# zjkang/Relation-DETR

Hardware: AMD Instinct MI355X
Metric: images/sec @ 800×1333, 300 queries, R50 4-level; achieved HBM GB/s (higher is better)
Workload: dtype bf16; 1 GPU; relation_detr_resnet50_800_1333 transformer stack from feature pyramids: 6 encoder layers (MSDA self-attn, S=22323, 4 levels) + two-stage top-k + 6 decoder layers (relation-biased self-attn + MSDA cross-attn + box refinement) + top-300 detections; backbone/neck excluded; batch_per_gpu=4, global_batch=4, queries=900, levels=4, launch=hipGraph replay, streams=2, gemm_tuning=False, parallelism=image-parallel x1

## Files before the change

include/relation_detr_amd.h:

```cpp
#ifndef RELATION_DETR_AMD_H
#define RELATION_DETR_AMD_H

#include <stdint.h>

#ifdef __cplusplus
extern "C" {
#endif

#define RDETR_ABI_VERSION 3

typedef enum rdetr_status {
    RDETR_OK = 0,
    RDETR_ERR_INVALID_ARG = -1,
    RDETR_ERR_UNSUPPORTED = -2,
    RDETR_ERR_LAUNCH = -3
} rdetr_status;

int rdetr_abi_version(void);
const char *rdetr_status_string(int status);

int rdetr_msda_forward_f32(const float *value, const int64_t *spatial_shapes, const int64_t *level_start_index,
                           const float *sampling_loc, const float *attn_weight, int B, int S, int H, int D,
                           int L, int Nq, int P, float *out, void *stream);

// ... 219 lines not shown
int rdetr_query_pos_inproj_k256_bf16(const uint16_t *emb, long long lde, const uint16_t *query, long long ldq, const uint16_t *pw1a,
                                     const uint16_t *pw1b, const uint16_t *b1, const uint16_t *pw2, const uint16_t *b2, const uint16_t *pv1,
                                     const uint16_t *c1, const uint16_t *pv2, const uint16_t *c2, const uint16_t *pwq, const uint16_t *pwk,
                                     const uint16_t *pwv, const uint16_t *bias, long long M, uint16_t *out_pos, uint16_t *out_qpp,
                                     uint16_t *out_qk, long long ldqk, uint16_t *out_v, long long ldv, void *stream);

int rdetr_encoder_proj_k256_bf16(const uint16_t *x, long long ldx, const uint16_t *xq, long long ldq, const uint16_t *pwv,
                                 const uint16_t *bv, const uint16_t *pwq, const uint16_t *bq, const uint8_t *row_mask, int B, int S,
                                 int q_cols, uint16_t *out_hm, uint16_t *out_q, void *stream);

int rdetr_detections_from_topk(const float *score, const long long *index, const float *boxes, const long long *image_sizes, int B,
                               int N, int C, int K, float *out, void *stream);

int rdetr_scaled_pos(const void *a, const void *scale, const void *query, long long n, int is_bf16, void *pos, void *qp, void *stream);

int rdetr_decoder_reference(const float *reference, const float *valid_ratios, int B, int N, int L, int F, float temperature,
                            float scale, float *ref_in, void *emb, int emb_is_bf16, void *stream);

int rdetr_pyramid_points(const unsigned char *const *level_masks, const int *level_hw, int L, int B, const unsigned char *pad_mask,
                         int keep_is_bf16, float *valid_ratios, float *reference, float *logit, void *keep, void *stream);
int rdetr_nchw_to_tokens(const void *src, const void *add_vec, int is_bf16, int B, int C, int P,
                         long long out_image_stride, long long ld_out, void *out, void *stream);
int rdetr_nchw_levels_to_tokens(const void *const *level_src, const void *const *level_vec, const int *level_pixels, int L,
                                int is_bf16, int B, int C, long long out_image_stride, long long ld_out, void *out, void *stream);

int rdetr_linear_k256_bf16(const uint16_t *x, long long ldx, const uint16_t *w, const uint16_t *bias, long long M, int N,
                           int relu, uint16_t *out, long long ldo, void *stream);

int rdetr_linear_pack_k256_bf16(const uint16_t *w, uint16_t *packed, void *stream);
int rdetr_linear_ln_k256_bf16(const uint16_t *x, long long ldx, const uint16_t *packed, const uint16_t *bias,
                              const uint16_t *residual, long long ldr, const uint16_t *gamma, const uint16_t *beta, float eps,
                              long long M, uint16_t *out, long long ldo, void *stream);

int rdetr_ffn_k256_pack_bf16(const uint16_t *w1, const uint16_t *w2, int F, uint16_t *packed, void *stream);
int rdetr_ffn_k256_bf16(const uint16_t *x, long long ldx, const uint16_t *packed, const uint16_t *b1, const uint16_t *b2,
                        long long M, int F, uint16_t *out, long long ldo, void *stream);
int rdetr_ffn_ln_k256_bf16(const uint16_t *x, long long ldx, const uint16_t *packed, const uint16_t *b1, const uint16_t *b2,
                           const uint16_t *gamma, const uint16_t *beta, float eps, const uint16_t *pos, long long ldp,
                           long long M, int F, uint16_t *out, long long ldo, uint16_t *out2, long long ldo2, void *stream);
int rdetr_ffn_k256_train_bf16(const uint16_t *x, long long ldx, const uint16_t *packed, const uint16_t *b1, const uint16_t *b2,
                              long long M, int F, uint16_t *out, long long ldo, uint16_t *hid, long long ldh, void *stream);
int rdetr_ffn_k256_backward_bf16(const uint16_t *dy, long long lddy, const uint16_t *packed_t, const uint16_t *hid, long long ldh,
                                 long long M, int F, uint16_t *dh, long long ldd, uint16_t *dx, long long lddx, void *stream);
int rdetr_ffn_k256_pack_f32(const float *w1, long long w1_row_stride, long long w1_col_stride, const float *w2,
                            long long w2_row_stride, long long w2_col_stride, const float *b1, const float *b2, int F,
                            uint16_t *packed, uint16_t *biases_bf16, void *stream);
int rdetr_ffn_k256_train_xf32_bf16(const float *x, long long ldx, const uint16_t *packed, const uint16_t *b1, const uint16_t *b2,
                                   long long M, int F, uint16_t *out, long long ldo, uint16_t *hid, long long ldh, uint16_t *xlp,
                                   long long ldxl, void *stream);
int rdetr_ffn_k256_backward_dxf32_bf16(const uint16_t *dy, long long lddy, const uint16_t *packed_t, const uint16_t *hid,
                                       long long ldh, long long M, int F, uint16_t *dh, long long ldd, float *dx, long long lddx,
                                       void *stream);

int rdetr_match_cost_f32(const float *logits, long long ld_logits, const float *boxes, long long ld_boxes, const float *gt_boxes,
                         const int *gt_labels, const int *gt_count, int R, int B, int N, int C, int Gmax, float alpha, float gamma,
                         float w_class, float w_bbox, float w_giou, float *cost, void *stream);
int rdetr_match_cost_bf16(const uint16_t *logits, long long ld_logits, const float *boxes, long long ld_boxes, const float *gt_boxes,
                          const int *gt_labels, const int *gt_count, int R, int B, int N, int C, int Gmax, float alpha, float gamma,
                          float w_class, float w_bbox, float w_giou, float *cost, void *stream);
long long rdetr_set_loss_workspace_bytes(int R, int N);
int rdetr_set_loss_f32(const float *logits, long long ld_logits, const float *boxes, long long ld_boxes, const int *match,
                       const float *gt_boxes, const int *gt_labels, int R, int B, int N, int C, int Gmax, int n_split, float inv_norm_a,
                       float inv_norm_b, float alpha, float gamma, void *ws, long long ws_bytes, float *sums, float *dlogits,
                       float *dbox_l1, float *dbox_giou, void *stream);
int rdetr_set_loss_bf16(const uint16_t *logits, long long ld_logits, const float *boxes, long long ld_boxes, const int *match,
                        const float *gt_boxes, const int *gt_labels, int R, int B, int N, int C, int Gmax, int n_split, float inv_norm_a,
// ... 43 lines not shown
```

relation_detr_amd/_lib.py:

```python
from __future__ import annotations

import ctypes
import os

_HERE = os.path.dirname(os.path.abspath(__file__))
LIB_PATH = os.environ.get("RDETR_LIB_PATH") or os.path.join(_HERE, "librelation_detr_amd.so")

_c_int, _c_float, _vp, _c_ll = ctypes.c_int, ctypes.c_float, ctypes.c_void_p, ctypes.c_longlong
_c_ull = ctypes.c_ulonglong

SIGNATURES = {
    "rdetr_abi_version": [],
    "rdetr_status_string": [_c_int],
    "rdetr_msda_fast_path": [_c_int] * 4,
    "rdetr_msda_levels_window_ok": [_vp, _vp, _c_int, _c_ll],
    "rdetr_msda_forward_f32": [_vp] * 5 + [_c_int] * 7 + [_vp, _vp],
    "rdetr_msda_forward_bf16": [_vp] * 5 + [_c_int] * 7 + [_vp, _vp],
    "rdetr_msda_forward_fused_f32": [_vp] * 6 + [_c_int] * 8 + [_vp, _vp],
    "rdetr_msda_forward_fused_bf16": [_vp] * 6 + [_c_int] * 8 + [_vp, _vp],
    "rdetr_msda_forward_fused_ex_f32": [_vp] * 4 + [_c_int, _vp, _c_int, _vp, _c_int, _vp] + [_c_int] * 7 + [_vp, _vp],
    "rdetr_msda_forward_fused_ex_bf16": [_vp] * 4 + [_c_int, _vp, _c_int, _vp, _c_int, _vp] + [_c_int] * 7 + [_vp, _vp],
    "rdetr_msda_forward_opt_bf16": [_vp, _c_int] + [_vp] * 4 + [_c_int] * 8 + [_vp, _vp],
    "rdetr_msda_forward_sweep_bf16": [_vp, _c_int] + [_vp] * 4 + [_c_int] * 7 + [_vp, _vp],
    "rdetr_msda_forward_resident_bf16": [_vp] * 5 + [_c_int] * 7 + [_vp, _vp],
# ... 15 lines not shown
    "rdetr_relation_bias_backward_f32": [_vp] * 4 + [_c_int] * 5 + [_c_float] * 3 + [_vp] * 4,
    "rdetr_bias_softmax_f32": [_vp] * 3 + [_c_int] * 3 + [_vp],
    "rdetr_relation_attention_bf16": [_vp] * 3 + [_c_int] * 3 + [_vp, _vp] + [_c_int] * 5 + [_c_float, _vp, _c_int, _vp],
    "rdetr_relation_attention_train_bf16": [_vp] * 3 + [_c_int] * 3 + [_vp, _vp] + [_c_int] * 5 + [_c_float, _vp, _c_int, _vp, _vp],
    "rdetr_relation_attention_backward_workspace_bytes": [_c_int] * 3,
    "rdetr_relation_attention_backward_bf16": [_vp] * 3 + [_c_int] * 3 + [_vp, _c_int, _vp, _vp, _c_int, _vp, _vp] + [_c_int] * 5
                                              + [_c_float, _vp, _c_ll] + [_vp, _c_int] * 3 + [_vp, _vp],
    "rdetr_relation_attention_boxes_bf16": [_vp] * 3 + [_c_int] * 3 + [_vp] * 5 + [_c_int] * 6 + [_c_float] * 4 + [_vp, _c_int, _vp],
    "rdetr_relation_attention_boxes_train_bf16": [_vp] * 3 + [_c_int] * 3 + [_vp] * 5 + [_c_int] * 6 + [_c_float] * 4
                                                 + [_vp, _c_int, _vp, _vp],
    "rdetr_relation_attention_boxes_backward_workspace_bytes": [_c_int] * 4,
    "rdetr_relation_attention_boxes_backward_bf16": [_vp] * 3 + [_c_int] * 3 + [_vp, _c_int, _vp, _vp, _c_int] + [_vp] * 5 + [_c_int] * 6
                                                    + [_c_float] * 4 + [_vp, _c_ll] + [_vp, _c_int] * 3 + [_vp, _vp, _vp],
    "rdetr_box_refine_f32": [_vp, _c_int, _vp, _c_ll, _c_float, _vp, _vp],
    "rdetr_sine_pos_embed": [_vp, _c_ll, _c_int, _c_int, _c_float, _c_float, _vp, _c_int, _vp],
    "rdetr_zero_masked_rows": [_vp, _vp, _c_ll, _c_int, _c_ll, _vp],
    "rdetr_row_max": [_vp, _c_int, _c_ll, _c_int, _c_ll, _vp, _vp],
    "rdetr_topk_workspace_bytes": [_c_int, _c_int, _c_int],
    "rdetr_topk": [_vp, _c_int, _c_int, _c_int, _c_int, _vp, _vp, _vp, _vp],
    "rdetr_box_head_k256_bf16": [_vp, _c_ll, _vp, _c_ll, _vp, _vp, _vp, _vp, _vp, _vp, _vp, _c_int, _c_float, _c_ll, _vp, _vp, _vp],
    "rdetr_box_head_cls_k256_bf16": [_vp, _c_ll, _vp, _c_ll, _vp, _vp, _vp, _vp, _vp, _vp, _vp, _c_int, _c_float, _vp, _vp, _c_int, _c_ll,
                                     _vp, _vp, _vp, _c_ll, _vp],
    "rdetr_query_pos_k256_bf16": [_vp, _c_ll, _vp, _c_ll] + [_vp] * 9 + [_c_ll, _vp, _vp, _vp],
    "rdetr_query_pos_inproj_k256_bf16": [_vp, _c_ll, _vp, _c_ll] + [_vp] * 13 + [_c_ll, _vp, _vp, _vp, _c_ll, _vp, _c_ll, _vp],
    "rdetr_encoder_proj_k256_bf16": [_vp, _c_ll, _vp, _c_ll] + [_vp] * 5 + [_c_int, _c_int, _c_int, _vp, _vp, _vp],
    "rdetr_detections_from_topk": [_vp, _vp, _vp, _vp, _c_int, _c_int, _c_int, _c_int, _vp, _vp],
    "rdetr_scaled_pos": [_vp, _vp, _vp, _c_ll, _c_int, _vp, _vp, _vp],
    "rdetr_decoder_reference": [_vp, _vp, _c_int, _c_int, _c_int, _c_int, _c_float, _c_float, _vp, _vp, _c_int, _vp],
    "rdetr_pyramid_points": [_vp, _vp, _c_int, _c_int, _vp, _c_int, _vp, _vp, _vp, _vp, _vp],
    "rdetr_linear_k256_bf16": [_vp, _c_ll, _vp, _vp, _c_ll, _c_int, _c_int, _vp, _c_ll, _vp],
    "rdetr_linear_k256_hm_bf16": [_vp, _c_ll, _vp, _vp, _vp, _c_int, _c_int, _vp, _vp],
    "rdetr_linear_pack_k256_bf16": [_vp, _vp, _vp],
    "rdetr_linear_ln_k256_bf16": [_vp, _c_ll, _vp, _vp, _vp, _c_ll, _vp, _vp, _c_float, _c_ll, _vp, _c_ll, _vp],
    "rdetr_ffn_k256_pack_bf16": [_vp, _vp, _c_int, _vp, _vp],
    "rdetr_ffn_k256_bf16": [_vp, _c_ll, _vp, _vp, _vp, _c_ll, _c_int, _vp, _c_ll, _vp],
    "rdetr_ffn_ln_k256_bf16": [_vp, _c_ll, _vp, _vp, _vp, _vp, _vp, _c_float, _vp, _c_ll, _c_ll, _c_int, _vp, _c_ll, _vp, _c_ll, _vp],
    "rdetr_ffn_k256_train_bf16": [_vp, _c_ll, _vp, _vp, _vp, _c_ll, _c_int, _vp, _c_ll, _vp, _c_ll, _vp],
    "rdetr_ffn_k256_backward_bf16": [_vp, _c_ll, _vp, _vp, _c_ll, _c_ll, _c_int, _vp, _c_ll, _vp, _c_ll, _vp],
    "rdetr_ffn_k256_pack_f32": [_vp, _c_ll, _c_ll, _vp, _c_ll, _c_ll, _vp, _vp, _c_int, _vp, _vp, _vp],
    "rdetr_ffn_k256_train_xf32_bf16": [_vp, _c_ll, _vp, _vp, _vp, _c_ll, _c_int, _vp, _c_ll, _vp, _c_ll, _vp, _c_ll, _vp],
    "rdetr_ffn_k256_backward_dxf32_bf16": [_vp, _c_ll, _vp, _vp, _c_ll, _c_ll, _c_int, _vp, _c_ll, _vp, _c_ll, _vp],
    "rdetr_nchw_to_tokens": [_vp, _vp, _c_int, _c_int, _c_int, _c_int, _c_ll, _c_ll, _vp, _vp],
    "rdetr_nchw_levels_to_tokens": [_vp, _vp, _vp, _c_int, _c_int, _c_int, _c_int, _c_ll, _c_ll, _vp, _vp],
    "rdetr_add_layernorm_f32": [_vp] * 4 + [_c_ll, _c_int, _c_float, _vp, _vp],
    "rdetr_add_layernorm_bf16": [_vp] * 4 + [_c_ll, _c_int, _c_float, _vp, _vp],
    "rdetr_add_layernorm_strided_f32": [_vp] * 4 + [_c_ll, _c_int, _c_ll, _c_ll, _c_ll, _c_float, _vp, _vp],
    "rdetr_add_layernorm_strided_bf16": [_vp] * 4 + [_c_ll, _c_int, _c_ll, _c_ll, _c_ll, _c_float, _vp, _vp],
    "rdetr_add_layernorm_pos_f32": [_vp] * 5 + [_c_ll, _c_int] + [_c_ll] * 5 + [_c_float, _vp, _vp, _vp],
    "rdetr_add_layernorm_pos_bf16": [_vp] * 5 + [_c_ll, _c_int] + [_c_ll] * 5 + [_c_float, _vp, _vp, _vp],
    "rdetr_add_layernorm_train_f32": [_vp] * 4 + [_c_ll, _c_int, _c_ll, _c_ll, _c_ll, _c_float, _vp, _vp, _vp],
    "rdetr_add_layernorm_train_bf16": [_vp] * 4 + [_c_ll, _c_int, _c_ll, _c_ll, _c_ll, _c_float, _vp, _vp, _vp],
    "rdetr_add_layernorm_backward_workspace_bytes": [_c_ll],
    "rdetr_add_layernorm_backward_f32": [_vp, _c_ll] * 3 + [_vp, _vp, _c_ll, _c_int, _vp, _c_ll] + [_vp] * 4,
    "rdetr_add_layernorm_backward_bf16": [_vp, _c_ll] * 3 + [_vp, _vp, _c_ll, _c_int, _vp, _c_ll] + [_vp] * 4,
    "rdetr_add_layernorm_train_mixed": [_vp, _c_int, _c_ll, _vp, _c_int, _c_ll, _vp, _vp, _c_ll, _c_int, _c_float, _vp, _c_ll, _vp, _vp],
    "rdetr_add_layernorm_backward_mixed": [_vp, _c_ll, _vp, _c_int, _c_ll, _vp, _c_int, _c_ll, _vp, _vp, _c_ll, _c_int, _vp, _c_ll]
                                          + [_vp] * 5,
    "rdetr_match_cost_f32": [_vp, _c_ll, _vp, _c_ll, _vp, _vp, _vp] + [_c_int] * 5 + [_c_float] * 5 + [_vp, _vp],
    "rdetr_match_cost_bf16": [_vp, _c_ll, _vp, _c_ll, _vp, _vp, _vp] + [_c_int] * 5 + [_c_float] * 5 + [_vp, _vp],
    "rdetr_set_loss_workspace_bytes": [_c_int, _c_int],
    "rdetr_set_loss_f32": [_vp, _c_ll, _vp, _c_ll, _vp, _vp, _vp] + [_c_int] * 6 + [_c_float] * 4 + [_vp, _c_ll] + [_vp] * 5,
    "rdetr_set_loss_bf16": [_vp, _c_ll, _vp, _c_ll, _vp, _vp, _vp] + [_c_int] * 6 + [_c_float] * 4 + [_vp, _c_ll] + [_vp] * 5,
    "rdetr_cdn_queries_f32": [_vp] * 3 + [_c_int] * 6 + [_c_float] * 2 + [_vp] * 5 + [_c_int, _c_ull] + [_vp] * 4,
    "rdetr_cdn_queries_bf16": [_vp] * 3 + [_c_int] * 6 + [_c_float] * 2 + [_vp] * 5 + [_c_int, _c_ull] + [_vp] * 4,
    "rdetr_cdn_mask": [_c_int] * 3 + [_vp, _vp],
    "rdetr_cdn_embed_backward_f32": [_vp, _vp] + [_c_int] * 3 + [_vp, _vp],
# ... 41 lines not shown
```

relation_detr_amd/ms_deform_attn.py:

```python
from __future__ import annotations

import math
import warnings

import torch
from torch import Tensor, nn

from . import amp_train, ln_train, msda_train_hm, ops
from . import options as _options


def sampling_locations(reference_points: Tensor, offsets: Tensor, spatial_shapes: Tensor, num_points: int) -> Tensor:
    last = reference_points.shape[-1]
    if last == 2:
        wh = spatial_shapes.flip(-1).to(offsets.dtype)
        return reference_points[:, :, None, :, None, :] + offsets / wh[None, None, None, :, None, :]
    if last == 4:
        centre = reference_points[:, :, None, :, None, :2]
        size = reference_points[:, :, None, :, None, 2:]
        return centre + offsets / num_points * size * 0.5
    raise ValueError("Last dim of reference_points must be 2 or 4, but get {} instead.".format(last))


class MultiScaleDeformableAttention(nn.Module):
    def __init__(self, embed_dim: int = 256, num_levels: int = 4, num_heads: int = 8, num_points: int = 4,
                 img2col_step: int = 64):
        super().__init__()
        if embed_dim % num_heads != 0:
            raise ValueError(
                "embed_dim must be divisible by num_heads, but got {} and {}".format(embed_dim, num_heads))
        head_dim = embed_dim // num_heads
        if head_dim & (head_dim - 1):
            warnings.warn("head_dim is not a power of two; the wave-per-query HIP kernel needs head_dim == 32, "
                          "other sizes run the generic kernel")
        self.im2col_step = img2col_step
        self.embed_dim = embed_dim
        self.num_heads = num_heads
        self.num_levels = num_levels
        self.num_points = num_points
        self.options = _options.get()
        self.sampling_offsets = nn.Linear(embed_dim, num_heads * num_levels * num_points * 2)
# ... 138 lines not shown
                and ops.msda_fast_path(self.num_heads, self.embed_dim // self.num_heads, self.num_levels, self.num_points)):
            core = ops.ms_deform_attn_forward_fused(
                v.to(core_dtype).contiguous(), spatial_shapes, level_start_index, offsets.to(core_dtype).contiguous(),
                logits.to(core_dtype).contiguous(), reference_points.float().contiguous())
        elif (needs_grad and self.options.msda_train_fused and v.is_cuda and core_dtype in (torch.float32, torch.bfloat16)
                and ops.msda_fast_path(self.num_heads, self.embed_dim // self.num_heads, self.num_levels, self.num_points)):
            core = ops.MultiScaleDeformableAttnFusedFunction.apply(
                v.to(core_dtype).contiguous(), spatial_shapes, level_start_index, offsets.to(core_dtype).contiguous(),
                logits.to(core_dtype).contiguous(), reference_points.float().contiguous())
        else:
            weights = logits.softmax(-1).view(*offsets.shape[:5])
            loc = sampling_locations(reference_points, offsets, spatial_shapes, self.num_points)
            core = ops.MultiScaleDeformableAttnFunction.apply(
                v.to(core_dtype).contiguous(), spatial_shapes, level_start_index, loc.float().contiguous(),
                weights.float().contiguous(), self.im2col_step)
        return self._output(core, vdt, post_norm)

    def _trains_head_major(self, query: Tensor, reference_points: Tensor, value: Tensor) -> bool:
        if not (self.options.msda_train_head_major and self.options.value_head_major and torch.is_grad_enabled() and value.is_cuda):
            return False
        so, aw, vp = self.sampling_offsets, self.attention_weights, self.value_proj
        if not (value.dtype == torch.bfloat16 and query.dtype == torch.bfloat16 and reference_points.shape[-1] == 2
                and query.shape[1] == value.shape[1] and value.shape[1] >= 4096 and value.dim() == 3 and query.shape[0] == value.shape[0]
                and all(m.weight.dtype == torch.bfloat16 for m in (so, aw, vp)) and so.bias is not None and aw.bias is not None
                and ops.msda_fast_path(self.num_heads, self.embed_dim // self.num_heads, self.num_levels, self.num_points)):
            return False
        return any(t.requires_grad for t in (query, value, reference_points, *so.parameters(), *aw.parameters(), *vp.parameters()))

    def _output(self, core: Tensor, vdt, post_norm) -> Tensor:
        if core.dtype != vdt:
            core = core.to(vdt)
        if post_norm is None:
            return self.output_proj(core)
        residual, norm = post_norm
        if (core.is_cuda and not torch.is_grad_enabled() and core.numel() // core.shape[-1] >= 16384
                and self.options.proj_ln and norm.weight is not None and norm.bias is not None
                and ops.linear_ln_k256_supported(core, self.output_proj.weight, residual)):
            return ops.linear_ln_k256(core, self.output_proj.weight, self.output_proj.bias, residual, norm.weight, norm.bias, norm.eps)
        out = self.output_proj(core)
        if out.is_cuda and not torch.is_grad_enabled() and out.dtype in (torch.float32, torch.bfloat16):
            return ops.add_layer_norm(out, residual, norm.weight, norm.bias, norm.eps)
        if (self.options.ln_train_fused and torch.is_grad_enabled()
                and (out.requires_grad or residual.requires_grad or (norm.weight is not None and norm.weight.requires_grad))):
            if ln_train.add_layer_norm_train_supported(out, residual, norm.weight, norm.bias):
                return ln_train.AddLayerNormFunction.apply(out, residual, norm.weight, norm.bias, norm.eps)
            if amp_train.autocast_bf16_active() and amp_train.add_layer_norm_mixed_supported(out, residual, norm.weight, norm.bias):
                return amp_train.AddLayerNormMixedFunction.apply(out, residual, norm.weight, norm.bias, norm.eps)
        return norm(residual + out)
```

relation_detr_amd/ops.py:

```python
from __future__ import annotations

import collections
import weakref
from typing import Optional, Tuple

import torch

from . import _lib


_KEEP: "collections.deque" = collections.deque(maxlen=64)


def _cptr(t: torch.Tensor) -> int:
    if t.is_contiguous():
        return t.data_ptr()
    c = t.contiguous()
    _KEEP.append(c)
    return c.data_ptr()


def _stream_ptr(t: torch.Tensor) -> int:
    return torch.cuda.current_stream(t.device).cuda_stream


def _require_device(*tensors: torch.Tensor) -> None:
    for t in tensors:
        if t is not None and not t.is_cuda:
            raise _lib.RdetrError(
                "relation_detr_amd operators need tensors on a ROCm device (got a CPU tensor); "
                "there is no CPU fallback on the product path")


def _require_contiguous(**named: torch.Tensor) -> None:
    for name, t in named.items():
        if t is not None and not t.is_contiguous():
            raise _lib.RdetrError(f"{name} tensor has to be contiguous")


_shape_cache: dict = {}

# ... 1303 lines not shown
    out2, ldp = None, 0
    if pos is not None:
        if tuple(pos.shape) != tuple(x.shape) or pos.dtype != x.dtype:
            raise _lib.RdetrError("ffn_ln_k256: pos must have x's shape and dtype")
        prows, _, ldp = _rows_view(pos, "ffn_ln_k256")
        if ldp % 8 or pos.data_ptr() % 16:
            raise _lib.RdetrError("ffn_ln_k256: pos rows must be 16-byte aligned")
        out2 = torch.empty(*x.shape[:-1], 256, dtype=x.dtype, device=x.device)
    packed = ffn_k256_packed_weights(w1, w2)
    st = _lib.load().rdetr_ffn_ln_k256_bf16(x.data_ptr(), ldx, packed.data_ptr(), _cptr(b1), _cptr(b2),
                                            _cptr(gamma), _cptr(beta), float(eps),
                                            None if pos is None else pos.data_ptr(), ldp, rows, F, out.data_ptr(), ldo,
                                            None if out2 is None else out2.data_ptr(), 256, _stream_ptr(x))
    _lib.check(st, "rdetr_ffn_ln_k256_bf16")
    return out if pos is None else (out, out2)


_LINEAR_PACKED = _PackedWeightCache()
_REL_PROJ_F32 = _PackedWeightCache()


def linear_ln_k256_supported(x: torch.Tensor, weight: torch.Tensor, residual: torch.Tensor) -> bool:
    if not (linear_k256_supported(x, weight) and tuple(weight.shape) == (256, 256) and residual.dtype == torch.bfloat16
            and residual.is_cuda and tuple(residual.shape) == tuple(x.shape)):
        return False
    try:
        _, _, ldr = _rows_view(residual, "linear_ln_k256")
    except _lib.RdetrError:
        return False
    return ldr % 8 == 0 and residual.data_ptr() % 16 == 0


def linear_ln_k256(x: torch.Tensor, weight: torch.Tensor, bias: Optional[torch.Tensor], residual: torch.Tensor,
                   gamma: torch.Tensor, beta: torch.Tensor, eps: float = 1e-5, out: Optional[torch.Tensor] = None) -> torch.Tensor:
    _require_device(x, weight, bias, residual, gamma, beta, out)
    if not linear_ln_k256_supported(x, weight, residual):
        raise _lib.RdetrError("linear_ln_k256: needs bf16 [..., 256] inputs with evenly strided 16-byte aligned rows and a [256, 256] weight")
    for t in (bias, gamma, beta):
        if t is not None and (t.dtype != torch.bfloat16 or t.numel() != 256):
            raise _lib.RdetrError("linear_ln_k256: bias / gamma / beta must be bf16 [256]")
    rows, _, ldx = _rows_view(x, "linear_ln_k256")
    _, _, ldr = _rows_view(residual, "linear_ln_k256")
    if out is None:
        out = torch.empty(x.shape, dtype=x.dtype, device=x.device)
    elif tuple(out.shape) != tuple(x.shape) or out.dtype != x.dtype:
        raise _lib.RdetrError("linear_ln_k256: out must have x's shape and dtype")
    orows, _, ldo = _rows_view(out, "linear_ln_k256")
    if orows != rows or ldo % 8 or out.data_ptr() % 16:
        raise _lib.RdetrError("linear_ln_k256: out rows must be 16-byte aligned")
    lib = _lib.load()
    def build():
        packed = torch.empty(256 * 256, dtype=torch.bfloat16, device=weight.device)
        _lib.check(lib.rdetr_linear_pack_k256_bf16(weight.data_ptr(), packed.data_ptr(), _stream_ptr(weight)), "rdetr_linear_pack_k256_bf16")
        if not torch.cuda.is_current_stream_capturing():
            torch.cuda.current_stream(weight.device).synchronize()
        return packed
    packed_w = _LINEAR_PACKED.get((weight,), build)
    st = lib.rdetr_linear_ln_k256_bf16(x.data_ptr(), ldx, packed_w.data_ptr(), None if bias is None else _cptr(bias),
                                       residual.data_ptr(), ldr, _cptr(gamma), _cptr(beta),
                                       float(eps), rows, out.data_ptr(), ldo, _stream_ptr(x))
    _lib.check(st, "rdetr_linear_ln_k256_bf16")
    return out
```

relation_detr_amd/self_attn.py:

```python
from __future__ import annotations

import math
from typing import Optional

import torch
from torch import Tensor, nn
from torch.nn import functional as F

from . import ops, options
from .attn_rel_train import RelationAttentionBoxesFunction
from .relation import DeferredRelationBias


class _BiasSoftmaxFunction(torch.autograd.Function):
    @staticmethod
    def forward(ctx, scores, bias, mask):
        probs = ops.bias_softmax_(scores, bias, mask)
        ctx.save_for_backward(probs)
        ctx.has_bias = bias is not None
        ctx.mark_dirty(scores)
        return probs

    @staticmethod
    @torch.autograd.function.once_differentiable
    def backward(ctx, grad):
        (p,) = ctx.saved_tensors
        gs = p * (grad - (grad * p).sum(-1, keepdim=True))
        return gs, (gs if ctx.has_bias else None), None


class RelationSelfAttention(nn.Module):

    def __init__(self, embed_dim: int, num_heads: int, dropout: float = 0.0, batch_first: bool = True):
        super().__init__()
        if not batch_first:
            raise NotImplementedError("the reference only uses batch_first=True (relation_transformer.py:406-408)")
        if embed_dim % num_heads:
            raise ValueError("embed_dim must be divisible by num_heads")
        self.embed_dim, self.num_heads, self.head_dim = embed_dim, num_heads, embed_dim // num_heads
        self.dropout = dropout
        self.batch_first = True
        self.in_proj_weight = nn.Parameter(torch.empty(3 * embed_dim, embed_dim))
        self.in_proj_bias = nn.Parameter(torch.zeros(3 * embed_dim))
        self.out_proj = nn.Linear(embed_dim, embed_dim)
        nn.init.xavier_uniform_(self.in_proj_weight)
        nn.init.zeros_(self.out_proj.bias)
        self.options = options.get()

    def forward(self, query: Tensor, key: Tensor, value: Tensor, attn_mask: Optional[Tensor] = None,
                need_weights: bool = False, key_padding_mask: Optional[Tensor] = None, projected=None):
        if need_weights or key_padding_mask is not None:
            raise NotImplementedError("need_weights / key_padding_mask are not used on this path")
        B, N, C = query.shape
        M = key.shape[1]
        H, d = self.num_heads, self.head_dim
        v = None
        if (projected is not None and key is query and not torch.is_grad_enabled() and query.dtype == torch.bfloat16
                and all(torch.is_tensor(t) and t.dtype == torch.bfloat16 and t.device == query.device for t in projected)
                and tuple(projected[0].shape) == (B, N, 2 * C) and tuple(projected[1].shape) == (B, M, C)):
            qk, v = projected
            q, k = qk[..., :C], qk[..., C:]
        elif key is query:
            qk = F.linear(query, self.in_proj_weight[:2 * C], self.in_proj_bias[:2 * C])
            q, k = qk[..., :C], qk[..., C:]
        else:
            q = F.linear(query, self.in_proj_weight[:C], self.in_proj_bias[:C])
            k = F.linear(key, self.in_proj_weight[C:2 * C], self.in_proj_bias[C:2 * C])
        if v is None:
            v = F.linear(value, self.in_proj_weight[2 * C:], self.in_proj_bias[2 * C:])
        needs_grad = torch.is_grad_enabled() and (q.requires_grad or k.requires_grad or v.requires_grad)
        if isinstance(attn_mask, DeferredRelationBias):
            rel = attn_mask
            conv = rel.module.pos_proj[0]
            if (q.is_cuda and q.dtype == torch.bfloat16 and d == 32 and H == 8 and rel.module.num_pos_feats == 16 and not needs_grad
                    and not (torch.is_grad_enabled() and conv.weight.requires_grad)
                    and tuple(rel.src_boxes.shape) == (B, N, 4) and tuple(rel.tgt_boxes.shape) == (B, M, 4)
                    and (rel.attn_mask is None or rel.attn_mask.dtype == torch.bool and tuple(rel.attn_mask.shape) == (N, M))):
                ctx = ops.relation_attention_boxes(q, k, v, H, rel.src_boxes, rel.tgt_boxes, conv.weight, conv.bias, rel.attn_mask,
                                                   1.0 / math.sqrt(d), rel.module.num_pos_feats, rel.module.temperature,
                                                   rel.module.scale)
                return self.out_proj(ctx), None
            if (self.options.rel_train_fused and torch.is_grad_enabled() and (needs_grad or conv.weight.requires_grad)
                    and q.is_cuda and q.dtype == torch.bfloat16 and k.dtype == torch.bfloat16 and v.dtype == torch.bfloat16
                    and d == 32 and H == 8 and rel.module.num_pos_feats == 16 and (self.dropout == 0.0 or not self.training)
                    and tuple(rel.src_boxes.shape) == (B, N, 4) and tuple(rel.tgt_boxes.shape) == (B, M, 4)
                    and (rel.attn_mask is None or rel.attn_mask.dtype == torch.bool and tuple(rel.attn_mask.shape) == (N, M))):
                packed = key is query
                ctx = RelationAttentionBoxesFunction.apply(
                    qk if packed else q, None if packed else k, v, rel.src_boxes, rel.tgt_boxes, conv.weight, conv.bias, rel.attn_mask,
                    H, 1.0 / math.sqrt(d), rel.module.num_pos_feats, rel.module.temperature, rel.module.scale)
                return self.out_proj(ctx), None
            attn_mask = rel.materialize()
        if (needs_grad and self.options.attn_train_fused and q.is_cuda and q.dtype == torch.bfloat16 and k.dtype == torch.bfloat16
                and v.dtype == torch.bfloat16 and d == 32 and (self.dropout == 0.0 or not self.training)
                and (attn_mask is None or attn_mask.dtype == torch.bool and tuple(attn_mask.shape) == (N, M)
                     or attn_mask.dtype != torch.bool and attn_mask.numel() == B * H * N * M)):
            is_bool = attn_mask is not None and attn_mask.dtype == torch.bool
            bias = None if attn_mask is None or is_bool else attn_mask.float().reshape(B * H, N, M)
            mask = attn_mask if is_bool else None
            if key is query:
                ctx = ops.RelationAttentionFunction.apply(qk, None, v, bias, mask, H, 1.0 / math.sqrt(d))
            else:
                ctx = ops.RelationAttentionFunction.apply(q, k, v, bias, mask, H, 1.0 / math.sqrt(d))
            return self.out_proj(ctx), None
        if (q.is_cuda and q.dtype == torch.bfloat16 and d == 32 and not needs_grad
                and (attn_mask is None or attn_mask.dtype == torch.bool and attn_mask.dim() == 2
                     or attn_mask.dtype != torch.bool and attn_mask.numel() == B * H * N * M)):
            is_bool = attn_mask is not None and attn_mask.dtype == torch.bool
            ctx = ops.relation_attention(q, k, v, H, None if attn_mask is None or is_bool else attn_mask.float(),
                                         attn_mask if is_bool else None, 1.0 / math.sqrt(d))
            return self.out_proj(ctx), None
        q = (q * (1.0 / math.sqrt(d))).view(B, N, H, d).transpose(1, 2).contiguous()
        k = k.view(B, M, H, d).transpose(1, 2).contiguous()
        v = v.view(B, M, H, d).transpose(1, 2).contiguous()
        scores = torch.matmul(q, k.transpose(-1, -2)).float().reshape(B * H, N, M).contiguous()
        bias = mask = None
        if attn_mask is not None:
            if attn_mask.dtype == torch.bool:
                if attn_mask.dim() != 2:
                    raise NotImplementedError("boolean attn_mask must be [N, N]")
                mask = attn_mask
            else:
                bias = attn_mask.float().reshape(B * H, N, M)
        probs = _BiasSoftmaxFunction.apply(scores, bias, mask)
        if self.dropout > 0.0 and self.training:
            probs = F.dropout(probs, self.dropout)
        ctx = torch.matmul(probs.view(B, H, N, M).to(v.dtype), v).transpose(1, 2).reshape(B, N, C)
        return self.out_proj(ctx), None
```

relation_detr_amd/transformer.py:

```python
from __future__ import annotations

import math
from typing import List, Sequence

import torch
from torch import Tensor, nn
from torch.nn import functional as F

from . import amp_train, ffn_train, ln_train, ops
from . import options as _options
from .ms_deform_attn import MultiScaleDeformableAttention
from .relation import PositionRelationEmbedding
from .self_attn import RelationSelfAttention


def inverse_sigmoid(x: Tensor, eps: float = 1e-3) -> Tensor:
    x = x.clamp(min=0, max=1)
    return torch.log(x.clamp(min=eps) / (1 - x).clamp(min=eps))


def refine_boxes(delta: Tensor, reference: Tensor) -> Tensor:
    if delta.is_cuda and reference.dtype == torch.float32 and not (torch.is_grad_enabled() and delta.requires_grad):
        from . import ops
        return ops.box_refine(delta, reference)
    return (delta.float() + inverse_sigmoid(reference)).sigmoid()


def sine_pos_embed(pos: Tensor, num_pos_feats: int = 128, temperature: float = 10000.0,
                   scale: float = 2 * math.pi) -> Tensor:
    k = torch.arange(num_pos_feats // 2, dtype=torch.float32, device=pos.device)
    dim_t = temperature ** (k * 2 / num_pos_feats)
    ang = pos.unsqueeze(-1) * scale / dim_t
    emb = torch.stack((ang.sin(), ang.cos()), dim=-1).flatten(-2)
    return torch.cat((emb[..., 1:2, :], emb[..., 0:1, :], emb[..., 2:, :]), dim=-2).flatten(-2)


def add_norm(norm: nn.LayerNorm, x: Tensor, residual: Tensor = None, out: Tensor = None, opts: "_options.Options" = None) -> Tensor:
    needs_grad = torch.is_grad_enabled() and (x.requires_grad or norm.weight.requires_grad or
                                              (residual is not None and residual.requires_grad))
    if x.is_cuda and not needs_grad and x.dtype in (torch.float32, torch.bfloat16):
        from . import ops
        return ops.add_layer_norm(x, residual, norm.weight, norm.bias, norm.eps, out=out)
# ... 136 lines not shown
            for i, layer in enumerate(self.layers):
                last = i + 1 == self.num_layers
                res = layer(query, query_pos, reference_points, spatial_shapes, level_start_index, query_key_padding_mask,
                            out=stacked[..., (i + 1) * d:(i + 2) * d], query_plus_pos=qpp,
                            next_pos=query_pos if fuse_pos and not last else None)
                query, qpp = res if isinstance(res, tuple) else (res, None)
            return add_norm(fuse[3], fuse[2](linear_relu(fuse[0], stacked, self.options)), opts=self.options)
        outs = [query]
        for layer in self.layers:
            query = layer(query, query_pos, reference_points, spatial_shapes, level_start_index, query_key_padding_mask)
            outs.append(query)
        return add_norm(fuse[3], fuse[2](linear_relu(fuse[0], torch.cat(outs, -1), self.options)), opts=self.options)


class RelationTransformerDecoderLayer(nn.Module):
    def __init__(self, embed_dim=256, d_ffn=1024, n_heads=8, n_levels=4, n_points=4,
                 msda_cls=MultiScaleDeformableAttention, self_attn_cls=RelationSelfAttention):
        super().__init__()
        self.embed_dim, self.num_heads = embed_dim, n_heads
        self.options = _options.get()
        self.cross_attn = msda_cls(embed_dim, n_levels, n_heads, n_points)
        self.norm1 = nn.LayerNorm(embed_dim)
        self.self_attn = self_attn_cls(embed_dim, n_heads, dropout=0.0, batch_first=True)
        self.norm2 = nn.LayerNorm(embed_dim)
        self.linear1 = nn.Linear(embed_dim, d_ffn)
        self.linear2 = nn.Linear(d_ffn, embed_dim)
        self.norm3 = nn.LayerNorm(embed_dim)
        nn.init.xavier_uniform_(self.linear1.weight)
        nn.init.xavier_uniform_(self.linear2.weight)

    def forward(self, query, query_pos, reference_points, value, spatial_shapes, level_start_index, self_attn_mask=None,
                key_padding_mask=None, query_plus_pos=None, projected_value=None, projected=None):
        qp = query + query_pos if query_plus_pos is None else query_plus_pos
        attn = self.self_attn(query=qp, key=qp, value=query, attn_mask=self_attn_mask, need_weights=False,
                              **({} if projected is None else {"projected": projected}))[0]
        if (query.is_cuda and not torch.is_grad_enabled() and query.dtype in (torch.float32, torch.bfloat16)
                and query_pos.dtype == query.dtype and query_pos.shape == query.shape and self.options.decoder_ln_pos):
            query, cross_q = ops.add_layer_norm(attn, query, self.norm2.weight, self.norm2.bias, self.norm2.eps, pos=query_pos)
        else:
            query = add_norm(self.norm2, query, attn, opts=self.options)
            cross_q = query + query_pos
        cross = self.cross_attn(query=cross_q, reference_points=reference_points, value=value,
                                spatial_shapes=spatial_shapes, level_start_index=level_start_index,
                                key_padding_mask=key_padding_mask,
                                **({} if projected_value is None else {"projected_value": projected_value}))
        query = add_norm(self.norm1, query, cross, opts=self.options)
        return add_norm(self.norm3, query, feed_forward(self.linear1, self.linear2, query, self.options), opts=self.options)


class RelationTransformerDecoder(nn.Module):

    def __init__(self, layers: Sequence[RelationTransformerDecoderLayer], num_classes: int,
                 relation_cls=PositionRelationEmbedding):
        super().__init__()
        self.layers = nn.ModuleList(layers)
        self.num_layers = len(self.layers)
        self.embed_dim, self.num_heads = self.layers[0].embed_dim, self.layers[0].num_heads
        self.options = _options.get()
        d = self.embed_dim
        self.ref_point_head = MLP(2 * d, d, d, 2)
        self.query_scale = MLP(d, d, d, 2)
        self.class_head = nn.ModuleList(nn.Linear(d, num_classes) for _ in range(self.num_layers))
        self.bbox_head = nn.ModuleList(MLP(d, d, 4, 3) for _ in range(self.num_layers))
        self.norm = nn.LayerNorm(d)
        self.position_relation_embedding = relation_cls(16, self.num_heads)
        prior = -math.log((1 - 0.01) / 0.01)
        for head in self.class_head:
            nn.init.constant_(head.bias, prior)
        for head in self.bbox_head:
            nn.init.zeros_(head.layers[-1].weight)
            nn.init.zeros_(head.layers[-1].bias)

    def _batched_value_projection(self, value: Tensor):
        projs = [layer.cross_attn.value_proj for layer in self.layers]
        key = tuple((p.weight._version, p.bias._version, p.weight.data_ptr(), p.weight.dtype) for p in projs)
        cache = getattr(self, "_value_proj_cache", None)
        if cache is None or cache[0] != key:
            with torch.no_grad():
                cache = (key, torch.cat([p.weight for p in projs], 0).contiguous(), torch.cat([p.bias for p in projs], 0).contiguous())
# ... 301 lines not shown
```

Baseline: 1091 images/s.

## Fuse decoder out-projections with residual LayerNorm via small-row linear-LN kernel

Adds a new HIP kernel that computes a 256x256 linear projection, bias, residual add and LayerNorm for small row counts, and can also emit the normalised output plus a positional embedding. The decoder layer routes both the relation self-attention out_proj (with norm2 and query_pos) and the MSDA cross-attention output_proj (with norm1) through it when rows fit under a cap. The goal is to remove the separate GEMM, add+LayerNorm and pos-add launches and their intermediate HBM round trips in the decoder, where 3600 rows are too few for the existing large-M fused kernel. The cost is extra dispatch logic and a kernel specialised for K=256 with one 32-row tile per block.

```diff
diff --git a/include/relation_detr_amd.h b/include/relation_detr_amd.h
--- a/include/relation_detr_amd.h
+++ b/include/relation_detr_amd.h
@@ -275,6 +275,11 @@
                               const uint16_t *residual, long long ldr, const uint16_t *gamma, const uint16_t *beta, float eps,
                               long long M, uint16_t *out, long long ldo, void *stream);
 
+int rdetr_linear_ln_rows_bf16(const uint16_t *x, long long ldx, const uint16_t *packed, const uint16_t *bias,
+                              const uint16_t *residual, long long ldr, const uint16_t *gamma, const uint16_t *beta, float eps,
+                              const uint16_t *pos, long long ldp, long long M, uint16_t *out, long long ldo, uint16_t *out_pos,
+                              long long ldop, void *stream);
+
 int rdetr_ffn_k256_pack_bf16(const uint16_t *w1, const uint16_t *w2, int F, uint16_t *packed, void *stream);
 int rdetr_ffn_k256_bf16(const uint16_t *x, long long ldx, const uint16_t *packed, const uint16_t *b1, const uint16_t *b2,
                         long long M, int F, uint16_t *out, long long ldo, void *stream);
diff --git a/relation_detr_amd/_lib.py b/relation_detr_amd/_lib.py
--- a/relation_detr_amd/_lib.py
+++ b/relation_detr_amd/_lib.py
@@ -71,6 +71,7 @@
     "rdetr_linear_k256_hm_bf16": [_vp, _c_ll, _vp, _vp, _vp, _c_int, _c_int, _vp, _vp],
     "rdetr_linear_pack_k256_bf16": [_vp, _vp, _vp],
     "rdetr_linear_ln_k256_bf16": [_vp, _c_ll, _vp, _vp, _vp, _c_ll, _vp, _vp, _c_float, _c_ll, _vp, _c_ll, _vp],
+    "rdetr_linear_ln_rows_bf16": [_vp, _c_ll, _vp, _vp, _vp, _c_ll, _vp, _vp, _c_float, _vp, _c_ll, _c_ll, _vp, _c_ll, _vp, _c_ll, _vp],
     "rdetr_ffn_k256_pack_bf16": [_vp, _vp, _c_int, _vp, _vp],
     "rdetr_ffn_k256_bf16": [_vp, _c_ll, _vp, _vp, _vp, _c_ll, _c_int, _vp, _c_ll, _vp],
     "rdetr_ffn_ln_k256_bf16": [_vp, _c_ll, _vp, _vp, _vp, _vp, _vp, _c_float, _vp, _c_ll, _c_ll, _c_int, _vp, _c_ll, _vp, _c_ll, _vp],
diff --git a/relation_detr_amd/csrc/rowtail.hip b/relation_detr_amd/csrc/rowtail.hip
--- /dev/null
+++ b/relation_detr_amd/csrc/rowtail.hip
@@ -0,0 +1,196 @@
+#include "common.h"
+
+namespace rdetr {
+
+typedef __bf16 rt_bf16x8 __attribute__((ext_vector_type(8)));
+
+constexpr int kRtWaves = 8, kRtThreads = kRtWaves * 64;
+constexpr int kRtRows = 32;
+constexpr int kRtLd = 256 + 4;
+constexpr int kRtXImg = 2 * 8 * 64;
+
+struct RtFrags { u32x4 f[16]; };
+
+__device__ __forceinline__ float rt_half_sum(float v)
+{
+#pragma unroll
+    for (int o = 16; o >= 1; o >>= 1) v += __shfl_xor(v, o, 64);
+    return v;
+}
+
+__device__ __forceinline__ void rt_widen8(const u32x4 &r, float (&v)[8])
+{
+    v[0] = __builtin_bit_cast(float, r.x << 16); v[1] = __builtin_bit_cast(float, r.x & 0xffff0000u);
+    v[2] = __builtin_bit_cast(float, r.y << 16); v[3] = __builtin_bit_cast(float, r.y & 0xffff0000u);
+    v[4] = __builtin_bit_cast(float, r.z << 16); v[5] = __builtin_bit_cast(float, r.z & 0xffff0000u);
+    v[6] = __builtin_bit_cast(float, r.w << 16); v[7] = __builtin_bit_cast(float, r.w & 0xffff0000u);
+}
+
+__device__ __forceinline__ u32x4 rt_load8(const uint16_t *p) { return *reinterpret_cast<const u32x4 *>(p); }
+
+__device__ __forceinline__ void rt_store8(uint16_t *p, const float (&v)[8])
+{
+    *reinterpret_cast<u32x4 *>(p) = u32x4{pack_bf16x2(v[0], v[1]), pack_bf16x2(v[2], v[3]), pack_bf16x2(v[4], v[5]), pack_bf16x2(v[6], v[7])};
+}
+
+__device__ __forceinline__ void rt_normalise(float (&v)[8], const float (&g)[8], const float (&b)[8], float eps, float (&y)[8])
+{
+    float s = 0.f;
+#pragma unroll
+    for (int k = 0; k < 8; ++k) s += v[k];
+    const float mean = rt_half_sum(s) * (1.0f / 256.0f);
+    float sq = 0.f;
+#pragma unroll
+    for (int k = 0; k < 8; ++k) {
+        v[k] -= mean;
+        sq += v[k] * v[k];
+    }
+    const float rstd = 1.0f / sqrtf(rt_half_sum(sq) * (1.0f / 256.0f) + eps);
+#pragma unroll
+    for (int k = 0; k < 8; ++k) y[k] = v[k] * rstd * g[k] + b[k];
+}
+
+struct RtArgs {
+    const uint16_t *x, *packed, *bias, *res, *gamma, *beta, *pos;
+    uint16_t *out, *out_pos;
+    long long ldx, ldr, ldp, ldo, ldop, M;
+    float eps;
+};
+
+template <bool kPos>
+__global__ __launch_bounds__(kRtThreads) void linear_ln_rows_kernel(RtArgs a)
+{
+    __shared__ __attribute__((aligned(16))) u32x4 xs[kRtXImg];
+    __shared__ __attribute__((aligned(16))) float img[kRtRows * kRtLd];
+    const int tid = threadIdx.x, lane = tid & 63, wave = __builtin_amdgcn_readfirstlane(tid >> 6);
+    const int col = lane & 15, g = lane >> 4;
+    const long long row0 = (long long)blockIdx.x * kRtRows;
+
+    RtFrags w;
+    {
+        const u32x4 *wp = reinterpret_cast<const u32x4 *>(a.packed) + (size_t)wave * 16 * 64 + lane;
+#pragma unroll
+        for (int i = 0; i < 16; ++i) w.f[i] = wp[((i & 1) * 8 + (i >> 1)) * 64];
+    }
+    long long rr[2];
+    u32x4 xr[2];
+#pragma unroll
+    for (int cb = 0; cb < 2; ++cb) {
+        rr[cb] = row0 + 16 * cb + col < a.M ? row0 + 16 * cb + col : a.M - 1;
+        xr[cb] = rt_load8(a.x + rr[cb] * a.ldx + 32 * wave + 8 * g);
+    }
+    const int c0 = 32 * wave + 8 * g;
+    const int half = lane >> 5, c = (lane & 31) * 8;
+    u32x4 rv[2], pr[2];
+#pragma unroll
+    for (int cb = 0; cb < 2; ++cb) rv[cb] = rt_load8(a.res + rr[cb] * a.ldr + c0);
+    const u32x4 bq = a.bias ? rt_load8(a.bias + c0) : u32x4{0u, 0u, 0u, 0u};
+    const u32x4 gq = rt_load8(a.gamma + c), tq = rt_load8(a.beta + c);
+    if (kPos) {
+#pragma unroll
+        for (int i = 0; i < 2; ++i) {
+            const long long row = row0 + 16 * i + 2 * wave + half;
+            pr[i] = rt_load8(a.pos + (row < a.M ? row : a.M - 1) * a.ldp + c);
+        }
+    }
+    __builtin_amdgcn_sched_barrier(0);
+#pragma unroll
+    for (int cb = 0; cb < 2; ++cb) xs[(cb * 8 + wave) * 64 + lane] = xr[cb];
+    __syncthreads();
+
+    f32x4 acc[2][2];
+#pragma unroll
+    for (int e = 0; e < 2; ++e)
+#pragma unroll
+        for (int cb = 0; cb < 2; ++cb) acc[e][cb] = f32x4{0.f, 0.f, 0.f, 0.f};
+    {
+        const u32x4 *xi = xs + lane;
+        u32x4 xb[2][2];
+        xb[0][0] = xi[0];
+        xb[0][1] = xi[8 * 64];
+#pragma unroll
+        for (int s = 0; s < 8; ++s) {
+            if (s + 1 < 8) {
+                xb[(s + 1) & 1][0] = xi[(s + 1) * 64];
+                xb[(s + 1) & 1][1] = xi[(8 + s + 1) * 64];
+            }
+            __builtin_amdgcn_sched_barrier(0);
+#pragma unroll
+            for (int cb = 0; cb < 2; ++cb)
+#pragma unroll
+                for (int e = 0; e < 2; ++e)
+                    acc[e][cb] = __builtin_amdgcn_mfma_f32_16x16x32_bf16(__builtin_bit_cast(rt_bf16x8, w.f[2 * s + e]),
+                                                                         __builtin_bit_cast(rt_bf16x8, xb[s & 1][cb]), acc[e][cb], 0, 0, 0);
+            __builtin_amdgcn_sched_barrier(0);
+        }
+    }
+
+    {
+        float bb[8];
+        rt_widen8(bq, bb);
+#pragma unroll
+        for (int cb = 0; cb < 2; ++cb) {
+            float rf[8];
+            rt_widen8(rv[cb], rf);
+            const f32x4 lo = acc[0][cb], hi = acc[1][cb];
+            const float o[8] = {lo.x + bb[0], lo.y + bb[1], lo.z + bb[2], lo.w + bb[3], hi.x + bb[4], hi.y + bb[5], hi.z + bb[6], hi.w + bb[7]};
+            float s[8];
+#pragma unroll
+            for (int k = 0; k < 8; ++k) s[k] = bf16_bits_to_f32(f32_to_bf16_bits(o[k])) + rf[k];
+            float *dst = img + (16 * cb + col) * kRtLd + c0;
+            *reinterpret_cast<f32x4 *>(dst) = f32x4{s[0], s[1], s[2], s[3]};
+            *reinterpret_cast<f32x4 *>(dst + 4) = f32x4{s[4], s[5], s[6], s[7]};
+        }
+    }
+    __syncthreads();
+
+    float gm[8], bt[8];
+    rt_widen8(gq, gm);
+    rt_widen8(tq, bt);
+#pragma unroll
+    for (int i = 0; i < 2; ++i) {
+        const int lr = 16 * i + 2 * wave + half;
+        const long long row = row0 + lr;
+        const bool ok = row < a.M;
+        float v[8], y[8];
+        const f32x4 v0 = *reinterpret_cast<const f32x4 *>(img + lr * kRtLd + c), v1 = *reinterpret_cast<const f32x4 *>(img + lr * kRtLd + c + 4);
+        v[0] = v0.x; v[1] = v0.y; v[2] = v0.z; v[3] = v0.w; v[4] = v1.x; v[5] = v1.y; v[6] = v1.z; v[7] = v1.w;
+        rt_normalise(v, gm, bt, a.eps, y);
+        if (ok) rt_store8(a.out + row * a.ldo + c, y);
+        if (kPos && ok) {
+            float pv[8];
+            rt_widen8(pr[i], pv);
+#pragma unroll
+            for (int k = 0; k < 8; ++k) pv[k] += bf16_bits_to_f32(f32_to_bf16_bits(y[k]));
+            rt_store8(a.out_pos + row * a.ldop + c, pv);
+        }
+    }
+}
+
+}
+
+using namespace rdetr;
+
+extern "C" int rdetr_linear_ln_rows_bf16(const uint16_t *x, long long ldx, const uint16_t *packed, const uint16_t *bias,
+                                         const uint16_t *residual, long long ldr, const uint16_t *gamma, const uint16_t *beta, float eps,
+                                         const uint16_t *pos, long long ldp, long long M, uint16_t *out, long long ldo, uint16_t *out_pos,
+                                         long long ldop, void *stream)
+{
+    const bool has_pos = pos != nullptr;
+    if (M < 0 || ldx < 256 || ldr < 256 || ldo < 256 || (has_pos && (ldp < 256 || ldop < 256))) return RDETR_ERR_INVALID_ARG;
+    if ((ldx & 7) || (ldr & 7) || (ldo & 7) || (has_pos && ((ldp & 7) || (ldop & 7)))) return RDETR_ERR_UNSUPPORTED;
+    if (M == 0) return RDETR_OK;
+    if (!x || !packed || !residual || !gamma || !beta || !out || (has_pos && !out_pos)) return RDETR_ERR_INVALID_ARG;
+    auto al = [](const void *p) { return reinterpret_cast<uintptr_t>(p) % 16 == 0; };
+    if (!al(x) || !al(packed) || !al(bias) || !al(residual) || !al(gamma) || !al(beta) || !al(out) || (has_pos && (!al(pos) || !al(out_pos))))
+        return RDETR_ERR_UNSUPPORTED;
+    const long long nblk = (M + kRtRows - 1) / kRtRows;
+    if (nblk > 0x7fffffffll) return RDETR_ERR_UNSUPPORTED;
+    const RtArgs a = {x, packed, bias, residual, gamma, beta, pos, out, out_pos, ldx, ldr, ldp, ldo, ldop, M, eps};
+    hipStream_t st = static_cast<hipStream_t>(stream);
+    if (has_pos)
+        hipLaunchKernelGGL(linear_ln_rows_kernel<true>, dim3((unsigned)nblk), dim3(kRtThreads), 0, st, a);
+    else
+        hipLaunchKernelGGL(linear_ln_rows_kernel<false>, dim3((unsigned)nblk), dim3(kRtThreads), 0, st, a);
+    return launch_status();
+}
diff --git a/relation_detr_amd/ms_deform_attn.py b/relation_detr_amd/ms_deform_attn.py
--- a/relation_detr_amd/ms_deform_attn.py
+++ b/relation_detr_amd/ms_deform_attn.py
@@ -6,7 +6,7 @@
 import torch
 from torch import Tensor, nn
 
-from . import amp_train, ln_train, msda_train_hm, ops
+from . import amp_train, ln_train, msda_train_hm, ops, rowtail
 from . import options as _options
 
 
@@ -211,8 +211,9 @@
             core = core.to(vdt)
         if post_norm is None:
             return self.output_proj(core)
-        residual, norm = post_norm
-        if (core.is_cuda and not torch.is_grad_enabled() and core.numel() // core.shape[-1] >= 16384
+        residual, norm = post_norm[:2]
+        rows = core.numel() // core.shape[-1]
+        if (core.is_cuda and not torch.is_grad_enabled() and (rows >= 16384 or (len(post_norm) == 3 and rowtail.takes(rows)))
                 and self.options.proj_ln and norm.weight is not None and norm.bias is not None
                 and ops.linear_ln_k256_supported(core, self.output_proj.weight, residual)):
             return ops.linear_ln_k256(core, self.output_proj.weight, self.output_proj.bias, residual, norm.weight, norm.bias, norm.eps)
diff --git a/relation_detr_amd/ops.py b/relation_detr_amd/ops.py
--- a/relation_detr_amd/ops.py
+++ b/relation_detr_amd/ops.py
@@ -6,7 +6,7 @@
 
 import torch
 
-from . import _lib
+from . import _lib, rowtail
 
 
 _KEEP: "collections.deque" = collections.deque(maxlen=64)
@@ -1376,14 +1376,20 @@
 
 
 def linear_ln_k256(x: torch.Tensor, weight: torch.Tensor, bias: Optional[torch.Tensor], residual: torch.Tensor,
-                   gamma: torch.Tensor, beta: torch.Tensor, eps: float = 1e-5, out: Optional[torch.Tensor] = None) -> torch.Tensor:
+                   gamma: torch.Tensor, beta: torch.Tensor, eps: float = 1e-5, out: Optional[torch.Tensor] = None,
+                   extra: Optional[dict] = None) -> torch.Tensor:
     _require_device(x, weight, bias, residual, gamma, beta, out)
     if not linear_ln_k256_supported(x, weight, residual):
         raise _lib.RdetrError("linear_ln_k256: needs bf16 [..., 256] inputs with evenly strided 16-byte aligned rows and a [256, 256] weight")
+    rows, _, ldx = _rows_view(x, "linear_ln_k256")
+    if rowtail.takes(rows):
+        return rowtail.linear_ln_rows(x, weight, bias, residual, gamma, beta, eps, out, extra, rows_view=_rows_view,
+                                      packed=_packed_k256(weight), keep=_KEEP)
+    if extra:
+        raise _lib.RdetrError(f"linear_ln_k256: `extra` is not supported above {rowtail.MAX_ROWS} rows")
     for t in (bias, gamma, beta):
         if t is not None and (t.dtype != torch.bfloat16 or t.numel() != 256):
             raise _lib.RdetrError("linear_ln_k256: bias / gamma / beta must be bf16 [256]")
-    rows, _, ldx = _rows_view(x, "linear_ln_k256")
     _, _, ldr = _rows_view(residual, "linear_ln_k256")
     if out is None:
         out = torch.empty(x.shape, dtype=x.dtype, device=x.device)
diff --git a/relation_detr_amd/rowtail.py b/relation_detr_amd/rowtail.py
--- /dev/null
+++ b/relation_detr_amd/rowtail.py
@@ -0,0 +1,67 @@
+from __future__ import annotations
+
+from typing import Optional
+
+import torch
+
+from . import _lib
+
+MAX_ROWS = 28800
+
+
+def takes(rows: int) -> bool:
+    return rows <= MAX_ROWS
+
+
+def _vector(t: Optional[torch.Tensor], name: str, keep) -> Optional[int]:
+    if t is None:
+        return None
+    if t.dtype != torch.bfloat16 or t.numel() != 256:
+        raise _lib.RdetrError(f"linear_ln_k256: {name} must be bf16 [256]")
+    t = t.detach()
+    if not t.is_contiguous() or t.data_ptr() % 16:
+        t = t.clone(memory_format=torch.contiguous_format)
+        keep.append(t)
+    return t.data_ptr()
+
+
+def _rows(t: torch.Tensor, rows: int, what: str, rows_view):
+    r, C, ld = rows_view(t, "linear_ln_k256")
+    if r != rows or C != 256 or ld % 8 or t.data_ptr() % 16 or t.dtype != torch.bfloat16:
+        raise _lib.RdetrError(f"linear_ln_k256: {what} must be bf16 [..., 256] with one row per input row, 16-byte aligned rows")
+    return ld
+
+
+def linear_ln_rows(x, weight, bias, residual, gamma, beta, eps, out, extra, *, rows_view, packed, keep):
+    rows, _, ldx = rows_view(x, "linear_ln_k256")
+    ldr = _rows(residual, rows, "residual", rows_view)
+    if out is None:
+        out = torch.empty(x.shape, dtype=x.dtype, device=x.device)
+    elif tuple(out.shape) != tuple(x.shape):
+        raise _lib.RdetrError("linear_ln_k256: out must have x's shape and dtype")
+    ldo = _rows(out, rows, "out", rows_view)
+    pos = out_pos = None
+    ldp = ldop = 0
+    if extra:
+        unknown = set(extra) - {"pos", "out_plus_pos", "out"}
+        if unknown:
+            raise _lib.RdetrError(f"linear_ln_k256: unknown extra keys {sorted(unknown)}")
+        pos = extra.get("pos")
+        if pos is not None:
+            if not pos.is_cuda or tuple(pos.shape) != tuple(x.shape):
+                raise _lib.RdetrError("linear_ln_k256: extra['pos'] must be a device tensor of x's shape")
+            ldp = _rows(pos, rows, "extra['pos']", rows_view)
+            out_pos = extra.get("out_plus_pos")
+            if out_pos is None:
+                out_pos = torch.empty(x.shape, dtype=x.dtype, device=x.device)
+            ldop = _rows(out_pos, rows, "extra['out_plus_pos']", rows_view)
+    st = _lib.load().rdetr_linear_ln_rows_bf16(
+        x.data_ptr(), ldx, packed.data_ptr(), _vector(bias, "bias", keep), residual.data_ptr(), ldr, _vector(gamma, "gamma", keep),
+        _vector(beta, "beta", keep), float(eps), None if pos is None else pos.data_ptr(), ldp, rows, out.data_ptr(), ldo,
+        None if out_pos is None else out_pos.data_ptr(), ldop, torch.cuda.current_stream(x.device).cuda_stream)
+    _lib.check(st, "rdetr_linear_ln_rows_bf16")
+    if extra is not None:
+        extra["out"] = out
+        if pos is not None:
+            extra["out_plus_pos"] = out_pos
+    return out
diff --git a/relation_detr_amd/self_attn.py b/relation_detr_amd/self_attn.py
--- a/relation_detr_amd/self_attn.py
+++ b/relation_detr_amd/self_attn.py
@@ -7,7 +7,7 @@
 from torch import Tensor, nn
 from torch.nn import functional as F
 
-from . import ops, options
+from . import ops, options, rowtail
 from .attn_rel_train import RelationAttentionBoxesFunction
 from .relation import DeferredRelationBias
 
@@ -48,7 +48,7 @@
         self.options = options.get()
 
     def forward(self, query: Tensor, key: Tensor, value: Tensor, attn_mask: Optional[Tensor] = None,
-                need_weights: bool = False, key_padding_mask: Optional[Tensor] = None, projected=None):
+                need_weights: bool = False, key_padding_mask: Optional[Tensor] = None, projected=None, post_norm=None):
         if need_weights or key_padding_mask is not None:
             raise NotImplementedError("need_weights / key_padding_mask are not used on this path")
         B, N, C = query.shape
@@ -79,7 +79,7 @@
                 ctx = ops.relation_attention_boxes(q, k, v, H, rel.src_boxes, rel.tgt_boxes, conv.weight, conv.bias, rel.attn_mask,
                                                    1.0 / math.sqrt(d), rel.module.num_pos_feats, rel.module.temperature,
                                                    rel.module.scale)
-                return self.out_proj(ctx), None
+                return self._inference_output(ctx, post_norm), None
             if (self.options.rel_train_fused and torch.is_grad_enabled() and (needs_grad or conv.weight.requires_grad)
                     and q.is_cuda and q.dtype == torch.bfloat16 and k.dtype == torch.bfloat16 and v.dtype == torch.bfloat16
                     and d == 32 and H == 8 and rel.module.num_pos_feats == 16 and (self.dropout == 0.0 or not self.training)
@@ -109,7 +109,7 @@
             is_bool = attn_mask is not None and attn_mask.dtype == torch.bool
             ctx = ops.relation_attention(q, k, v, H, None if attn_mask is None or is_bool else attn_mask.float(),
                                          attn_mask if is_bool else None, 1.0 / math.sqrt(d))
-            return self.out_proj(ctx), None
+            return self._inference_output(ctx, post_norm), None
         q = (q * (1.0 / math.sqrt(d))).view(B, N, H, d).transpose(1, 2).contiguous()
         k = k.view(B, M, H, d).transpose(1, 2).contiguous()
         v = v.view(B, M, H, d).transpose(1, 2).contiguous()
@@ -127,3 +127,13 @@
             probs = F.dropout(probs, self.dropout)
         ctx = torch.matmul(probs.view(B, H, N, M).to(v.dtype), v).transpose(1, 2).reshape(B, N, C)
         return self.out_proj(ctx), None
+
+    def _inference_output(self, ctx: Tensor, post_norm) -> Tensor:
+        if post_norm is not None and self.options.proj_ln:
+            residual, norm, extra = post_norm
+            proj = self.out_proj
+            if (type(norm) is nn.LayerNorm and norm.elementwise_affine and norm.bias is not None and proj.bias is not None
+                    and rowtail.takes(ctx.numel() // ctx.shape[-1]) and ops.linear_ln_k256_supported(ctx, proj.weight, residual)
+                    and all(p.dtype == torch.bfloat16 for p in (proj.bias, norm.weight, norm.bias))):
+                return ops.linear_ln_k256(ctx, proj.weight, proj.bias, residual, norm.weight, norm.bias, norm.eps, extra=extra)
+        return self.out_proj(ctx)
diff --git a/relation_detr_amd/transformer.py b/relation_detr_amd/transformer.py
--- a/relation_detr_amd/transformer.py
+++ b/relation_detr_amd/transformer.py
@@ -7,7 +7,7 @@
 from torch import Tensor, nn
 from torch.nn import functional as F
 
-from . import amp_train, ffn_train, ln_train, ops
+from . import amp_train, ffn_train, ln_train, ops, rowtail
 from . import options as _options
 from .ms_deform_attn import MultiScaleDeformableAttention
 from .relation import PositionRelationEmbedding
@@ -210,19 +210,32 @@
     def forward(self, query, query_pos, reference_points, value, spatial_shapes, level_start_index, self_attn_mask=None,
                 key_padding_mask=None, query_plus_pos=None, projected_value=None, projected=None):
         qp = query + query_pos if query_plus_pos is None else query_plus_pos
+        ln_pos = (query.is_cuda and not torch.is_grad_enabled() and query.dtype in (torch.float32, torch.bfloat16)
+                  and query_pos.dtype == query.dtype and query_pos.shape == query.shape and self.options.decoder_ln_pos)
+        tails = (query.is_cuda and not torch.is_grad_enabled() and query.dtype == torch.bfloat16 and query.shape[-1] == 256
+                 and self.options.proj_ln and rowtail.takes(query.numel() // 256))
+        post = {"pos": query_pos} if tails and ln_pos and type(self.self_attn) is RelationSelfAttention else None
         attn = self.self_attn(query=qp, key=qp, value=query, attn_mask=self_attn_mask, need_weights=False,
-                              **({} if projected is None else {"projected": projected}))[0]
-        if (query.is_cuda and not torch.is_grad_enabled() and query.dtype in (torch.float32, torch.bfloat16)
-                and query_pos.dtype == query.dtype and query_pos.shape == query.shape and self.options.decoder_ln_pos):
+                              **({} if projected is None else {"projected": projected}),
+                              **({} if post is None else {"post_norm": (query, self.norm2, post)}))[0]
+        if post is not None and "out" in post:
+            query, cross_q = attn, post["out_plus_pos"]
+        elif ln_pos:
             query, cross_q = ops.add_layer_norm(attn, query, self.norm2.weight, self.norm2.bias, self.norm2.eps, pos=query_pos)
         else:
             query = add_norm(self.norm2, query, attn, opts=self.options)
             cross_q = query + query_pos
-        cross = self.cross_attn(query=cross_q, reference_points=reference_points, value=value,
-                                spatial_shapes=spatial_shapes, level_start_index=level_start_index,
-                                key_padding_mask=key_padding_mask,
-                                **({} if projected_value is None else {"projected_value": projected_value}))
-        query = add_norm(self.norm1, query, cross, opts=self.options)
+        if tails and type(self.cross_attn).forward is MultiScaleDeformableAttention.forward:
+            query = self.cross_attn(query=cross_q, reference_points=reference_points, value=value,
+                                    spatial_shapes=spatial_shapes, level_start_index=level_start_index,
+                                    key_padding_mask=key_padding_mask, post_norm=(query, self.norm1, True),
+                                    **({} if projected_value is None else {"projected_value": projected_value}))
+        else:
+            cross = self.cross_attn(query=cross_q, reference_points=reference_points, value=value,
+                                    spatial_shapes=spatial_shapes, level_start_index=level_start_index,
+                                    key_padding_mask=key_padding_mask,
+                                    **({} if projected_value is None else {"projected_value": projected_value}))
+            query = add_norm(self.norm1, query, cross, opts=self.options)
         return add_norm(self.norm3, query, feed_forward(self.linear1, self.linear2, query, self.options), opts=self.options)
 
 
```

After: 1112 images/s (median of 6 runs). 1.02x the previous value.
